# DHDev0/Stochastic-muzero

Measured on NVIDIA B200. Metric: mcts_simulations_per_sec, higher is better.
Workload: dtype bf16

## Files before the change

stochastic-muzero_b200/csrc/smz_net_bf16.cu:

```cuda
#include <cuda_bf16.h>
#include <cuda_runtime.h>
#include <stdio.h>
#include <stdlib.h>
#include <string.h>

#include "../../include/smz.h"
#include "smz_net_bf16.h"
#include "smz_tc_ptx.cuh"
#include "smz_tree_dev.cuh"

namespace {

using namespace smz_tc;

constexpr int TM = 128;
constexpr int NTHREADS = 512;
constexpr int TN = 128;
constexpr int KMAX = 128;
constexpr int MAXL = 24;
constexpr int A_BYTES = TM * KMAX * 2;
constexpr int W_BYTES = TN * KMAX * 2;
constexpr int CHUNK_A = TM * 16;
constexpr int CHUNK_W = TN * 16;
constexpr int POL_OFF = 64;
// ... 620 lines not shown
  tc_fence_before();
  __syncthreads();
  if (warp == 0) {
    asm volatile("tcgen05.dealloc.cta_group::1.sync.aligned.b32 %0, %1;" ::"r"(tmem), "r"(2 * TN) : "memory");
  }
}

template <int NT>
struct SmemPipeN {
  alignas(1024) unsigned char a[NT][A_BYTES];
  alignas(1024) unsigned char w[2][W_BYTES];
  float bias[MAXL][TN];
  unsigned long long wbar[2];
  unsigned long long dbar[NT];
  unsigned long long bbar;
  unsigned int tmem_base;
  float4 part[2][4][TM];
  int rowidx[NT][TM];
};

template <int NT>
__global__ void __launch_bounds__(NPIPE, 1)
k_bf16_chain_pipeN(SmzArena a, Chain chain0, Chain chain1, Job job, int sim) {
  extern __shared__ unsigned char smem_raw[];
  SmemPipeN<NT>& sm = *reinterpret_cast<SmemPipeN<NT>*>((reinterpret_cast<uintptr_t>(smem_raw) + 1023) & ~uintptr_t(1023));
  constexpr int NR = 2;
  const int tid = threadIdx.x, warp = tid >> 5, lane = tid & 31;
  const bool is_issuer_warp = warp == NEPI / 32;
  const int r = (warp & 3) * 32 + lane;
  const int cb = (warp >> 2) & 3;
  const int group = blockIdx.x;
  const int nl = chain0.n_layers;

  auto load_weights = [&](const Chain& c, int l, int slot) {
    const unsigned bytes = (unsigned)c.layer[l].K * TN * 2;
    mbar_expect_tx(&sm.wbar[slot], bytes);
    bulk_g2s(sm.w[slot], c.layer[l].w, bytes, &sm.wbar[slot]);
  };
  if (tid == 0) {
    mbar_init(&sm.wbar[0], 1); mbar_init(&sm.wbar[1], 1);
#pragma unroll
    for (int t = 0; t < NT; ++t) mbar_init(&sm.dbar[t], 1);
    mbar_init(&sm.bbar, 1);
    asm volatile("fence.mbarrier_init.release.cluster;" ::: "memory");
    load_weights(chain0, 0, 0);
    load_weights(chain1, 0, 1);
  }
  __syncwarp();
  if (warp == 0) {
    asm volatile("tcgen05.alloc.cta_group::1.sync.aligned.shared::cta.b32 [%0], %1;" ::"r"(s32(&sm.tmem_base)), "r"(NT * TN)
                 : "memory");
    asm volatile("tcgen05.relinquish_alloc_permit.cta_group::1.sync.aligned;" ::: "memory");
  }
  smz_pdl_wait();
  smz_pdl_launch_dependents();
  int4 rec[NT];
  uint4 hrow[NT][2];
#pragma unroll
  for (int t = 0; t < NT; ++t) { rec[t] = make_int4(0, 0, 0, 0); hrow[t][0] = hrow[t][1] = make_uint4(0, 0, 0, 0); }
  if (!is_issuer_warp) {
#pragma unroll
    for (int t = 0; t < NT; ++t) {
      const size_t ri = (size_t)(sim & 1) * a.row_cap + (size_t)(NT * group + t) * TM + r;
      rec[t] = a.rows4[ri];
      if (a.xin) {
#pragma unroll
        for (int q = 0; q < 2; ++q) hrow[t][q] = a.xin[ri * 8 + cb * 2 + q];
      } else {
        rec[t].x = min(max(rec[t].x, 0), a.B - 1);
        rec[t].y = min(max(rec[t].y, 0), a.N);
        const __nv_bfloat16* src16 = reinterpret_cast<const __nv_bfloat16*>(a.hidden) + ((size_t)rec[t].y * a.B + rec[t].x) * SMZ_SP;
#pragma unroll
        for (int q = 0; q < 2; ++q) hrow[t][q] = *reinterpret_cast<const uint4*>(src16 + (cb * 2 + q) * 8);
      }
    }
  }
  const int count0 = a.branch_count[sim * 2], count1 = a.branch_count[sim * 2 + 1];
  const int top1 = a.row_top - count1;
  const int lo = NT * group * TM;
  const int branch = lo < count0 ? 0 : (lo + NT * TM > top1 ? 1 : -1);
  if (branch < 0) {
    if (tid == 0) {
      mbar_wait(&sm.wbar[0], 0);
      mbar_wait(&sm.wbar[1], 0);
    }
    tc_fence_before();
    __syncthreads();
    tc_fence_after();
    if (warp == 0)
      asm volatile("tcgen05.dealloc.cta_group::1.sync.aligned.b32 %0, %1;" ::"r"(sm.tmem_base), "r"(NT * TN) : "memory");
    return;
  }
  unsigned actm = 0;
#pragma unroll
  for (int t = 0; t < NT; ++t)
    if (branch ? lo + (t + 1) * TM > top1 : lo + t * TM < count0) actm |= 1u << t;
  const int t_last = 31 - __clz(actm);
  const Chain& ch = branch ? chain1 : chain0;
  if (tid == 0) {
    const unsigned bbytes = (unsigned)nl * TN * 4;
    mbar_expect_tx(&sm.bbar, bbytes);
    bulk_g2s(sm.bias, ch.bias, bbytes, &sm.bbar);
  }
  tc_fence_before();
  __syncthreads();
  tc_fence_after();
  const unsigned tmem = sm.tmem_base;

  if (is_issuer_warp) {
    unsigned nfill0 = 1u, nfill1 = 1u, nseen0 = 0u, nseen1 = 0u;
    const __nv_bfloat16 *res0 = branch ? nullptr : ch.layer[0].w, *res1 = branch ? ch.layer[0].w : nullptr;
    if (nl > 1) {
      const int s1 = branch ^ 1;
      mbar_wait(&sm.wbar[s1], 0);
      if (lane == 0) load_weights(ch, 1, s1);
      if (s1) { nseen1 = 1u; nfill1 = 2u; res1 = ch.layer[1].w; } else { nseen0 = 1u; nfill0 = 2u; res0 = ch.layer[1].w; }
      __syncwarp();
    }
    for (int l = 0; l < nl; ++l) {
      const int nk = ch.layer[l].K / 16;
      const int slot = (l + branch) & 1;
      const unsigned seen = slot ? nseen1 : nseen0;
      if (seen < (slot ? nfill1 : nfill0)) {
        mbar_wait(&sm.wbar[slot], seen & 1u);
        if (slot) ++nseen1; else ++nseen0;
      }
      const unsigned long long bd = umma_desc(s32(sm.w[slot]), CHUNK_W, 128);
#pragma unroll 1
      for (int t = 0; t < NT; ++t) {
        if (!((actm >> t) & 1u)) continue;
        const unsigned long long ad = umma_desc(s32(sm.a[t]), CHUNK_A, 128);
        const unsigned d = tmem + (unsigned)(t * TN);
        for (int c = 0; c < NR; ++c) {
          nb_sync(2 + 2 * t + c);
          tc_fence_after();
          if (elect_one()) {
#pragma unroll
            for (int k = 0; k < 8; ++k)
              if (k >= 4 * c && k < 4 * (c + 1) && k < nk)
                umma(d, ad + (unsigned long long)(k * ((2 * CHUNK_A) >> 4)), bd + (unsigned long long)(k * ((2 * CHUNK_W) >> 4)),
                     k > 0 ? 1u : 0u);
          }
          __syncwarp();
        }
        if (lane == 0) umma_commit(&sm.dbar[t]);
        __syncwarp();
      }
      if (l + 2 < nl && ((slot ? res1 : res0) != ch.layer[l + 2].w || job.stream_all)) {
        mbar_wait(&sm.dbar[t_last], l & 1);
        if (lane == 0) load_weights(ch, l + 2, slot);
        if (slot) { ++nfill1; res1 = ch.layer[l + 2].w; } else { ++nfill0; res0 = ch.layer[l + 2].w; }
        __syncwarp();
      }
    }
  } else {
#pragma unroll
    for (int t = 0; t < NT; ++t) {
      const int pos = lo + t * TM + r;
      const bool tact = (actm >> t) & 1u;
      const bool valid = tact && (branch ? pos >= top1 : pos < count0);
      if (cb == 0) sm.rowidx[t][r] = valid ? rec[t].x : -1;
      if (tact) {
        const int act = valid ? rec[t].z : -1;
#pragma unroll
        for (int q = 0; q < 2; ++q) a_store(sm.a[t], r, cb * 2 + q, valid ? hrow[t][q] : make_uint4(0, 0, 0, 0));
        for (int kc = cb; kc < ch.onehot_pad / 8; kc += 4) {
          unsigned w4[4] = {0, 0, 0, 0};
          if (valid && act >= kc * 8 && act < kc * 8 + 8) {
            const int j = act - kc * 8;
            w4[j >> 1] = (j & 1) ? 0x3F800000u : 0x00003F80u;
          }
          a_store(sm.a[t], r, 8 + kc, make_uint4(w4[0], w4[1], w4[2], w4[3]));
        }
      }
    }
    fence_async_smem();
#pragma unroll
    for (int t = 0; t < NT; ++t)
      if ((actm >> t) & 1u)
        for (int c = 0; c < NR; ++c) nb_arrive(2 + 2 * t + c);
    mbar_wait(&sm.bbar, 0);
    epi_sync();
    const float (*cbias)[TN] = sm.bias;
    const int S = job.S;

    for (int l = 0; l < nl; ++l) {
      const int kind = ch.layer[l].kind;
#pragma unroll 1
      for (int t = 0; t < NT; ++t) {
        if (!((actm >> t) & 1u)) continue;
        const int index_t = sm.rowidx[t][r];
        unsigned char* const A = sm.a[t];
        const unsigned lane_t = tmem + ((unsigned)((warp & 3) * 32) << 16) + (unsigned)(t * TN);
        mbar_wait(&sm.dbar[t], l & 1);
        __syncwarp();
        tc_fence_after();
        if (kind == LK_HIDDEN) {
          constexpr int SL = 32 / NR;
          constexpr int RC = TN / NR;
          const int j0 = cb * SL;
          unsigned raw[NR][SL];
#pragma unroll
          for (int c = 0; c < NR; ++c) tmem_ld16_nowait(lane_t + c * RC + j0, raw[c]);
          tmem_wait_ld();
#pragma unroll
          for (int c = 0; c < NR; ++c) {
            const float* bias = cbias[l] + c * RC + j0;
            float x[SL];
#pragma unroll
            for (int i = 0; i < SL; ++i) x[i] = elu_fast(__uint_as_float(raw[c][i]) + bias[i]);
#pragma unroll
            for (int q = 0; q < SL / 8; ++q)
              a_store(A, r, (c * RC + j0) / 8 + q,
                      make_uint4(pack_bf16(x[q * 8 + 0], x[q * 8 + 1]), pack_bf16(x[q * 8 + 2], x[q * 8 + 3]),
                                 pack_bf16(x[q * 8 + 4], x[q * 8 + 5]), pack_bf16(x[q * 8 + 6], x[q * 8 + 7])));
            fence_async_smem();
            if (c == NR - 1) tc_fence_before();
            nb_arrive(2 + 2 * t + c);
          }
        } else {
          const int c0 = cb * 32;
          const float* bias = cbias[l] + c0;
          float4 (*part)[TM] = sm.part[t & 1];
          uint4 pend[4];
          uint4* pend_dst = nullptr;
          float x[32];
          tmem_ld32(lane_t + c0, x);
#pragma unroll
          for (int i = 0; i < 32; ++i) x[i] += bias[i];
          const bool state_seg = (kind == LK_STATE || kind == LK_STATE_REWARD) && cb < 2;
          const bool soft_seg = (kind == LK_STATE_REWARD && cb >= 2) || (kind == LK_PRED && cb < 2);
          SoftPart sp{-1e30f, 0.f, 0.f};
          if (state_seg) {
            float lo_ = INFINITY, hi_ = -INFINITY;
#pragma unroll
            for (int i = 0; i < 32; ++i) { lo_ = fminf(lo_, x[i]); hi_ = fmaxf(hi_, x[i]); }
            part[cb][r] = make_float4(lo_, hi_, 0.f, 0.f);
          } else if (soft_seg) {
            sp = soft_part(x, c0 & 63, S);
            part[cb][r] = make_float4(sp.m, sp.z, sp.y, 0.f);
          }
          epi_sync();
          if (state_seg) {
            const float4 o = part[cb ^ 1][r];
            const float lo_ = fminf(part[cb][r].x, o.x), hi_ = fmaxf(part[cb][r].y, o.y);
            float scale = hi_ - lo_;
            if (scale < 1e-5f) scale += 1e-5f;
            const float inv = 1.f / scale;
#pragma unroll
            for (int i = 0; i < 32; ++i) x[i] = (x[i] - lo_) * inv;
            if (index_t >= 0 && job.hidden16_dst) pend_dst = reinterpret_cast<uint4*>(job.hidden16_dst + (size_t)index_t * SMZ_SP + c0);
#pragma unroll
            for (int q = 0; q < 4; ++q) {
              pend[q] = make_uint4(pack_bf16(x[q * 8 + 0], x[q * 8 + 1]), pack_bf16(x[q * 8 + 2], x[q * 8 + 3]),
                                   pack_bf16(x[q * 8 + 4], x[q * 8 + 5]), pack_bf16(x[q * 8 + 6], x[q * 8 + 7]));
              a_store(A, r, cb * 4 + q, pend[q]);
            }
          } else if (soft_seg && (cb & 1) == 0) {
            const float4 o = part[cb + 1][r];
            const float v = support_scalar(sp, SoftPart{o.x, o.y, o.z});
            float* dst = (kind == LK_PRED) ? job.value_dst : job.reward_dst;
            if (index_t >= 0 && dst) dst[index_t] = v;
          } else if (kind == LK_PRED && cb == 2) {
            const int n = ch.n_policy;
            float m = -1e30f, z = 0.f;
#pragma unroll
            for (int i = 0; i < 32; ++i) m = fmaxf(m, x[i]);
#pragma unroll
            for (int i = 0; i < 32; ++i) {
              x[i] = ex2f((x[i] - m) * 1.4426950408889634f);
              z += x[i];
            }
            if (index_t >= 0 && job.policy_dst) {
              float* dst = job.policy_dst + (size_t)index_t * job.pstride;
              const float inv = 1.f / z;
#pragma unroll
              for (int i = 0; i < 32; ++i)
                if (i < n) dst[i] = x[i] * inv;
            }
          }
          if (l + 1 < nl) {
            fence_async_smem();
            tc_fence_before();
            for (int c = 0; c < NR; ++c) nb_arrive(2 + 2 * t + c);
          }
          if (pend_dst) {
#pragma unroll
            for (int q = 0; q < 4; ++q) pend_dst[q] = pend[q];
          }
        }
      }
    }
  }
  tc_fence_before();
  __syncthreads();
  if (warp == 0) {
    asm volatile("tcgen05.dealloc.cta_group::1.sync.aligned.b32 %0, %1;" ::"r"(tmem), "r"(NT * TN) : "memory");
  }
}

constexpr int TM64 = 64;
constexpr int A64_BYTES = TM64 * KMAX * 2;
constexpr int CHUNK_A64 = TM64 * 16;
constexpr unsigned IDESC64 = (1u << 4) | (1u << 7) | (1u << 10) | ((unsigned)(TN >> 3) << 17) | ((unsigned)(TM64 >> 4) << 24);

struct Smem64 {
  alignas(1024) unsigned char a[A64_BYTES];
  alignas(1024) unsigned char w[2][W_BYTES];
  float bias[2][MAXL][TN];
  unsigned long long wbar[2];
  unsigned long long dbar[2];
  unsigned long long bbar;
  unsigned int tmem_base;
  int rowidx[TM64];
  float4 part[4][TM64];
};

__device__ __forceinline__ void umma64(unsigned tmem_d, unsigned long long adesc, unsigned long long bdesc, unsigned accum) {
  asm volatile(
      "{\n\t.reg .pred p;\n\t"
      "setp.ne.b32 p, %4, 0;\n\t"
      "tcgen05.mma.cta_group::1.kind::f16 [%0], %1, %2, %3, p;\n\t}" ::"r"(tmem_d),
      "l"(adesc), "l"(bdesc), "r"(IDESC64), "r"(accum)
      : "memory");
}
__device__ __forceinline__ void a64_store2(unsigned char* a, int row, int col, unsigned v) {
  asm volatile("st.shared.b32 [%0], %1;" ::"r"(s32(a + (col >> 3) * CHUNK_A64 + row * 16 + (col & 7) * 2)), "r"(v) : "memory");
}

template <int R0, bool HALF>
__device__ __forceinline__ void chain_m64_body(const SmzArena& a, const Chain& chain0, const Chain& chain1, const Job& job, int sim) {
  extern __shared__ unsigned char smem_raw[];
  Smem64& sm = *reinterpret_cast<Smem64*>((reinterpret_cast<uintptr_t>(smem_raw) + 1023) & ~uintptr_t(1023));
  constexpr int TV = HALF ? 32 : 64;
  const int tid = threadIdx.x, warp = tid >> 5, lane = tid & 31;
  const bool is_issuer_warp = warp == NEPI / 32;
  const int q = warp & 3;
  const int cb = (warp >> 2) & 3;
  const int rA = 16 * q + (lane >> 2), rB = rA + 8;
  const int cq = 2 * (lane & 3);

  const int tile = blockIdx.x;
  const int nl = chain0.n_layers;
  long long* tl = (job.timeline && blockIdx.x == 0 && lane == 0) ? job.timeline : nullptr;
  if (tl && tid == 0) tl[0] = clock64();

  auto load_weights = [&](const Chain& c, int l, int slot) {
    const unsigned bytes = (unsigned)c.layer[l].K * TN * 2;
    mbar_expect_tx(&sm.wbar[slot], bytes);
    bulk_g2s(sm.w[slot], c.layer[l].w, bytes, &sm.wbar[slot]);
  };
  if (tid == 0) {
    mbar_init(&sm.wbar[0], 1); mbar_init(&sm.wbar[1], 1);
    mbar_init(&sm.dbar[0], 1); mbar_init(&sm.dbar[1], 1);
    mbar_init(&sm.bbar, 1);
    asm volatile("fence.mbarrier_init.release.cluster;" ::: "memory");
    const unsigned bbytes = (unsigned)nl * TN * 4;
    mbar_expect_tx(&sm.bbar, 2 * bbytes);
    bulk_g2s(sm.bias[0], chain0.bias, bbytes, &sm.bbar);
    bulk_g2s(sm.bias[1], chain1.bias, bbytes, &sm.bbar);
    load_weights(chain0, 0, 0);
    load_weights(chain1, 0, 1);
  }
  __syncwarp();
  if (warp == 0) {
    asm volatile("tcgen05.alloc.cta_group::1.sync.aligned.shared::cta.b32 [%0], %1;" ::"r"(s32(&sm.tmem_base)), "r"(2 * TN)
                 : "memory");
    asm volatile("tcgen05.relinquish_alloc_permit.cta_group::1.sync.aligned;" ::: "memory");
  }
  smz_pdl_wait();
  smz_pdl_launch_dependents();
  smz_stamp_min(a.dbg, sim, 2);
  if (tl && tid == 0) tl[1 + 4 * MAXL] = clock64();
  const bool stager = HALF ? tid < 256 : !is_issuer_warp;
  const int srow = HALF ? (tid & 31) : (tid & 63), skc = HALF ? ((tid >> 5) & 7) : ((tid >> 6) & 7);
  const int mrow = HALF ? 16 * (srow >> 3) + (srow & 7) : srow;
  const int pos = tile * TV + srow;
  int4 rec = make_int4(0, 0, 0, 0);
  uint4 hrow = make_uint4(0, 0, 0, 0);
  if (stager) {
    const size_t ri = (size_t)(sim & 1) * a.row_cap + pos;
    rec = a.rows4[ri];
    if (a.xin) {
      hrow = a.xin[ri * 8 + skc];
    } else {
      rec.x = min(max(rec.x, 0), a.B - 1);
      rec.y = min(max(rec.y, 0), a.N);
      hrow = *reinterpret_cast<const uint4*>(reinterpret_cast<const __nv_bfloat16*>(a.hidden) +
                                             ((size_t)rec.y * a.B + rec.x) * SMZ_SP + skc * 8);
    }
  }
  const int count0 = a.branch_count[sim * 2], count1 = a.branch_count[sim * 2 + 1];
  const int top1 = a.row_top - count1;
  const int branch = tile * TV < count0 ? 0 : ((tile + 1) * TV > top1 ? 1 : -1);
  if (branch < 0) {
    if (tid == 0) {
      mbar_wait(&sm.bbar, 0);
      mbar_wait(&sm.wbar[0], 0);
      mbar_wait(&sm.wbar[1], 0);
    }
    tc_fence_before();
    __syncthreads();
    tc_fence_after();
    if (warp == 0)
      asm volatile("tcgen05.dealloc.cta_group::1.sync.aligned.b32 %0, %1;" ::"r"(sm.tmem_base), "r"(2 * TN) : "memory");
    return;
  }
  const Chain& ch = branch ? chain1 : chain0;
  tc_fence_before();
  __syncthreads();
  tc_fence_after();
  const unsigned tmem = sm.tmem_base;

  if (is_issuer_warp) {
    const unsigned long long ad = umma_desc(s32(sm.a), CHUNK_A64, 128);
    unsigned nfill0 = 1u, nfill1 = 1u, nseen0 = 0u, nseen1 = 0u;
    const __nv_bfloat16 *res0 = branch ? nullptr : ch.layer[0].w, *res1 = branch ? ch.layer[0].w : nullptr;
    if (nl > 1) {
      const int s1 = branch ^ 1;
      mbar_wait(&sm.wbar[s1], 0);
      if (lane == 0) load_weights(ch, 1, s1);
      if (s1) { nseen1 = 1u; nfill1 = 2u; res1 = ch.layer[1].w; } else { nseen0 = 1u; nfill0 = 2u; res0 = ch.layer[1].w; }
      __syncwarp();
    }
    for (int l = 0; l < nl; ++l) {
      const int nk = ch.layer[l].K / 16;
      const int slot = (l + branch) & 1;
      const unsigned seen = slot ? nseen1 : nseen0;
      if (seen < (slot ? nfill1 : nfill0)) {
        mbar_wait(&sm.wbar[slot], seen & 1u);
        if (slot) ++nseen1; else ++nseen0;
      }
      const unsigned long long bd = umma_desc(s32(sm.w[slot]), CHUNK_W, 128);
      const unsigned d = tmem + (unsigned)((l & 1) * TN);
      for (int c = 0; c < 2; ++c) {
        nb_sync(2 + c);
        if (tl && c == 1) tl[1 + l * 4 + 0] = clock64();
        if (tl && c == 0 && l == 3) tl[1 + 4 * MAXL + 10] = clock64();
        tc_fence_after();
        if (elect_one()) {
#pragma unroll
          for (int k = 0; k < 8; ++k)
            if (k >= (c ? R0 / 16 : 0) && k < (c ? 8 : R0 / 16) && k < nk)
              umma64(d, ad + (unsigned long long)(k * ((2 * CHUNK_A64) >> 4)), bd + (unsigned long long)(k * ((2 * CHUNK_W) >> 4)),
                     k > 0 ? 1u : 0u);
        }
        __syncwarp();
        if (tl && c == 0 && l == 3) tl[1 + 4 * MAXL + 11] = clock64();
      }
      if (lane == 0) umma_commit(&sm.dbar[l & 1]);
      if (tl) tl[1 + l * 4 + 1] = clock64();
      __syncwarp();
      if (l + 2 < nl && ((slot ? res1 : res0) != ch.layer[l + 2].w || job.stream_all)) {
        mbar_wait(&sm.dbar[l & 1], (l >> 1) & 1);
        if (lane == 0) load_weights(ch, l + 2, slot);
        if (slot) { ++nfill1; res1 = ch.layer[l + 2].w; } else { ++nfill0; res0 = ch.layer[l + 2].w; }
        __syncwarp();
      }
    }
  } else {
    {
      if (stager) {
        const bool valid = branch ? pos >= top1 : pos < count0;
        asm volatile("st.shared.v4.b32 [%0], {%1, %2, %3, %4};" ::"r"(s32(sm.a + skc * CHUNK_A64 + mrow * 16)), "r"(valid ? hrow.x : 0u),
                     "r"(valid ? hrow.y : 0u), "r"(valid ? hrow.z : 0u), "r"(valid ? hrow.w : 0u)
                     : "memory");
        if (skc < ch.onehot_pad / 8) {
          const int act = valid ? rec.z : -1;
          unsigned w4[4] = {0, 0, 0, 0};
          if (act >= skc * 8 && act < skc * 8 + 8) {
            const int j = act - skc * 8;
            w4[j >> 1] = (j & 1) ? 0x3F800000u : 0x00003F80u;
          }
          asm volatile("st.shared.v4.b32 [%0], {%1, %2, %3, %4};" ::"r"(s32(sm.a + (8 + skc) * CHUNK_A64 + mrow * 16)), "r"(w4[0]),
                       "r"(w4[1]), "r"(w4[2]), "r"(w4[3])
                       : "memory");
        }
        if (skc == 0) sm.rowidx[mrow] = valid ? rec.x : -1;
      } else {
        const int j = tid - 256;
        const int zrow = 16 * ((j >> 3) & 3) + 8 + (j & 7), zc = j >> 5;
#pragma unroll
        for (int h = 0; h < 2; ++h)
          asm volatile("st.shared.v4.b32 [%0], {%1, %1, %1, %1};" ::"r"(s32(sm.a + (zc + 8 * h) * CHUNK_A64 + zrow * 16)), "r"(0u)
                       : "memory");
        if (zc == 0) sm.rowidx[zrow] = -1;
      }
    }
    fence_async_smem();
    for (int c = 0; c < 2; ++c) nb_arrive(2 + c);
    mbar_wait(&sm.bbar, 0);
    epi_sync();
    const unsigned lane_t = tmem + ((unsigned)(q * 32) << 16);
    const int S = job.S;
    const int idxA = sm.rowidx[rA], idxB = HALF ? -1 : sm.rowidx[rB];
    const float (*bias)[TN] = sm.bias[branch];

    for (int l = 0; l < nl; ++l) {
      const int kind = ch.layer[l].kind;
      const unsigned dcol = (unsigned)((l & 1) * TN);
      constexpr int G0 = R0 / 32, G1 = (TN - R0) / 32;
      float2 bi[G0 + G1];
      if (kind == LK_HIDDEN) {
#pragma unroll
        for (int g = 0; g < G0 + G1; ++g)
          bi[g] = *reinterpret_cast<const float2*>(bias[l] + (g < G0 ? cb * 8 * G0 + g * 8 : R0 + cb * 8 * G1 + (g - G0) * 8) + cq);
      }
      mbar_wait(&sm.dbar[l & 1], (l >> 1) & 1);
      if (tl && warp == 0) tl[1 + l * 4 + 2] = clock64();
      __syncwarp();
      tc_fence_after();
      if (kind == LK_HIDDEN) {
        unsigned raw[4 * (G0 + G1)];
        if constexpr (R0 == 64) {
          tmem_ld16x256_x2(lane_t + dcol + cb * 16, raw);
          tmem_ld16x256_x2(lane_t + dcol + 64 + cb * 16, raw + 8);
        } else {
          tmem_ld16x256_x2(lane_t + dcol + cb * 24, raw);
          tmem_ld16x256_x1(lane_t + dcol + cb * 24 + 16, raw + 8);
          tmem_ld16x256_x1(lane_t + dcol + 96 + cb * 8, raw + 12);
        }
        tmem_wait_ld();
        const bool fine = tl && warp == 0 && l == 2;
        if (fine) tl[1 + 4 * MAXL + 2] = clock64();
        unsigned pa[G0 + G1], pb[G0 + G1];
        auto math = [&](int g) {
          const unsigned* rr = raw + 4 * g;
          pa[g] = pack_bf16(elu_fast(__uint_as_float(rr[0]) + bi[g].x), elu_fast(__uint_as_float(rr[1]) + bi[g].y));
          if constexpr (!HALF) pb[g] = pack_bf16(elu_fast(__uint_as_float(rr[2]) + bi[g].x), elu_fast(__uint_as_float(rr[3]) + bi[g].y));
        };
        if constexpr (HALF) {
#pragma unroll
          for (int g = 0; g < G0 + G1; ++g) math(g);
        }
#pragma unroll
        for (int c = 0; c < 2; ++c) {
          if constexpr (!HALF) {
#pragma unroll
            for (int g = 0; g < (c ? G1 : G0); ++g) math((c ? G0 : 0) + g);
          }
#pragma unroll
          for (int g = 0; g < (c ? G1 : G0); ++g) {
            const int col = (c ? R0 + cb * 8 * G1 : cb * 8 * G0) + g * 8 + cq;
            a64_store2(sm.a, rA, col, pa[(c ? G0 : 0) + g]);
            if constexpr (!HALF) a64_store2(sm.a, rB, col, pb[(c ? G0 : 0) + g]);
          }
          if (fine) tl[1 + 4 * MAXL + 3 + 3 * c] = clock64();
          fence_async_smem();
          if (c == 1) tc_fence_before();
          if (fine) tl[1 + 4 * MAXL + 4 + 3 * c] = clock64();
          nb_arrive(2 + c);
          if (fine) tl[1 + 4 * MAXL + 5 + 3 * c] = clock64();
        }
      } else {
        const int c0 = cb * 32;
        unsigned raw[16];
        tmem_ld16x256_x4(lane_t + dcol + c0, raw);
        tmem_wait_ld();
        float xa[8], xb[8];
#pragma unroll
        for (int g = 0; g < 4; ++g) {
          const float2 bi = *reinterpret_cast<const float2*>(bias[l] + c0 + g * 8 + cq);
          xa[2 * g] = __uint_as_float(raw[4 * g + 0]) + bi.x; xa[2 * g + 1] = __uint_as_float(raw[4 * g + 1]) + bi.y;
          if constexpr (!HALF) {
            xb[2 * g] = __uint_as_float(raw[4 * g + 2]) + bi.x; xb[2 * g + 1] = __uint_as_float(raw[4 * g + 3]) + bi.y;
          } else {
            xb[2 * g] = 0.f; xb[2 * g + 1] = 0.f;
          }
        }
        const bool state_seg = (kind == LK_STATE || kind == LK_STATE_REWARD) && cb < 2;
        const bool soft_seg = (kind == LK_STATE_REWARD && cb >= 2) || (kind == LK_PRED && cb < 2);
        SoftPart spa{-1e30f, 0.f, 0.f}, spb{-1e30f, 0.f, 0.f};
        if (state_seg) {
          float loa = INFINITY, hia = -INFINITY, lob = INFINITY, hib = -INFINITY;
#pragma unroll
          for (int i = 0; i < 8; ++i) {
            loa = fminf(loa, xa[i]); hia = fmaxf(hia, xa[i]);
            if constexpr (!HALF) { lob = fminf(lob, xb[i]); hib = fmaxf(hib, xb[i]); }
          }
#pragma unroll
          for (int off = 1; off <= 2; off <<= 1) {
            loa = fminf(loa, __shfl_xor_sync(0xffffffffu, loa, off)); hia = fmaxf(hia, __shfl_xor_sync(0xffffffffu, hia, off));
            if constexpr (!HALF) {
              lob = fminf(lob, __shfl_xor_sync(0xffffffffu, lob, off)); hib = fmaxf(hib, __shfl_xor_sync(0xffffffffu, hib, off));
            }
          }
          if ((lane & 3) == 0) {
            sm.part[cb][rA] = make_float4(loa, hia, 0.f, 0.f);
            if constexpr (!HALF) sm.part[cb][rB] = make_float4(lob, hib, 0.f, 0.f);
          }
        } else if (soft_seg) {
          float ma = -1e30f, mb = -1e30f;
#pragma unroll
          for (int i = 0; i < 8; ++i) { ma = fmaxf(ma, xa[i]); if constexpr (!HALF) mb = fmaxf(mb, xb[i]); }
          spa.m = ma; spb.m = mb;
#pragma unroll
          for (int g = 0; g < 4; ++g)
#pragma unroll
            for (int j = 0; j < 2; ++j) {
              const float pos_c = (float)(((c0 + g * 8 + cq + j) & 63) - S / 2);
              const float ea = ex2f((xa[2 * g + j] - ma) * 1.4426950408889634f);
              spa.z += ea; spa.y = fmaf(pos_c, ea, spa.y);
              if constexpr (!HALF) {
                const float eb = ex2f((xb[2 * g + j] - mb) * 1.4426950408889634f);
                spb.z += eb; spb.y = fmaf(pos_c, eb, spb.y);
              }
            }
          spa = soft_quad(spa);
          if constexpr (!HALF) spb = soft_quad(spb);
          if ((lane & 3) == 0) {
            sm.part[cb][rA] = make_float4(spa.m, spa.z, spa.y, 0.f);
            if constexpr (!HALF) sm.part[cb][rB] = make_float4(spb.m, spb.z, spb.y, 0.f);
          }
        }
        epi_sync();
        unsigned pend_a[4], pend_b[4];
        bool have_pend = false;
        if (state_seg) {
          const float4 oa = sm.part[cb ^ 1][rA], ma4 = sm.part[cb][rA];
          const float loa = fminf(ma4.x, oa.x), hia = fmaxf(ma4.y, oa.y);
          float sa = hia - loa;
          if (sa < 1e-5f) sa += 1e-5f;
          const float ia = 1.f / sa;
          float lob = 0.f, ib = 0.f;
          if constexpr (!HALF) {
            const float4 ob = sm.part[cb ^ 1][rB], mb4 = sm.part[cb][rB];
            lob = fminf(mb4.x, ob.x);
            float sb = fmaxf(mb4.y, ob.y) - lob;
            if (sb < 1e-5f) sb += 1e-5f;
            ib = 1.f / sb;
          }
#pragma unroll
          for (int g = 0; g < 4; ++g) {
            pend_a[g] = pack_bf16((xa[2 * g] - loa) * ia, (xa[2 * g + 1] - loa) * ia);
            a64_store2(sm.a, rA, c0 + g * 8 + cq, pend_a[g]);
            if constexpr (!HALF) {
              pend_b[g] = pack_bf16((xb[2 * g] - lob) * ib, (xb[2 * g + 1] - lob) * ib);
              a64_store2(sm.a, rB, c0 + g * 8 + cq, pend_b[g]);
            } else {
              pend_b[g] = 0u;
            }
          }
          have_pend = job.hidden16_dst != nullptr;
        } else if (soft_seg && (cb & 1) == 0) {
          if ((lane & 3) == 0) {
            float* dst = (kind == LK_PRED) ? job.value_dst : job.reward_dst;
            if (dst) {
              const float4 oa = sm.part[cb + 1][rA];
              if (idxA >= 0) dst[idxA] = support_scalar(spa, SoftPart{oa.x, oa.y, oa.z});
              if constexpr (!HALF) {
                const float4 ob = sm.part[cb + 1][rB];
                if (idxB >= 0) dst[idxB] = support_scalar(spb, SoftPart{ob.x, ob.y, ob.z});
              }
            }
          }
        } else if (kind == LK_PRED && cb == 2) {
          const int n = ch.n_policy;
          float ma = -1e30f, mb = -1e30f;
#pragma unroll
          for (int i = 0; i < 8; ++i) { ma = fmaxf(ma, xa[i]); if constexpr (!HALF) mb = fmaxf(mb, xb[i]); }
#pragma unroll
          for (int off = 1; off <= 2; off <<= 1) {
            ma = fmaxf(ma, __shfl_xor_sync(0xffffffffu, ma, off));
            if constexpr (!HALF) mb = fmaxf(mb, __shfl_xor_sync(0xffffffffu, mb, off));
          }
          float za = 0.f, zb = 0.f;
#pragma unroll
          for (int i = 0; i < 8; ++i) {
            xa[i] = ex2f((xa[i] - ma) * 1.4426950408889634f); za += xa[i];
            if constexpr (!HALF) { xb[i] = ex2f((xb[i] - mb) * 1.4426950408889634f); zb += xb[i]; }
          }
#pragma unroll
          for (int off = 1; off <= 2; off <<= 1) {
            za += __shfl_xor_sync(0xffffffffu, za, off);
            if constexpr (!HALF) zb += __shfl_xor_sync(0xffffffffu, zb, off);
          }
          if (job.policy_dst) {
            const float ia = 1.f / za, ib = HALF ? 0.f : 1.f / zb;
#pragma unroll
            for (int g = 0; g < 4; ++g)
#pragma unroll
              for (int j = 0; j < 2; ++j) {
                const int i = g * 8 + cq + j;
                if (i < n) {
                  if (idxA >= 0) job.policy_dst[(size_t)idxA * job.pstride + i] = xa[2 * g + j] * ia;
                  if constexpr (!HALF) {
                    if (idxB >= 0) job.policy_dst[(size_t)idxB * job.pstride + i] = xb[2 * g + j] * ib;
                  }
                }
              }
          }
        }
        if (l + 1 < nl) {
          fence_async_smem();
          tc_fence_before();
          for (int c = 0; c < 2; ++c) nb_arrive(2 + c);
        }
        if (have_pend) {
#pragma unroll
          for (int g = 0; g < 4; ++g) {
            if (idxA >= 0) *reinterpret_cast<unsigned*>(job.hidden16_dst + (size_t)idxA * SMZ_SP + c0 + g * 8 + cq) = pend_a[g];
            if constexpr (!HALF) {
              if (idxB >= 0) *reinterpret_cast<unsigned*>(job.hidden16_dst + (size_t)idxB * SMZ_SP + c0 + g * 8 + cq) = pend_b[g];
            }
          }
        }
      }
      if (tl && warp == 0) tl[1 + l * 4 + 3] = clock64();
    }
  }
  tc_fence_before();
  __syncthreads();
  smz_stamp_max(a.dbg, sim, 3);
  if (warp == 0) {
    asm volatile("tcgen05.dealloc.cta_group::1.sync.aligned.b32 %0, %1;" ::"r"(tmem), "r"(2 * TN) : "memory");
  }
}

template <int R0>
__global__ void __maxnreg__(80)
k_bf16_chain_m64(SmzArena a, Chain chain0, Chain chain1, Job job, int sim) {
  chain_m64_body<R0, false>(a, chain0, chain1, job, sim);
}
__global__ void __maxnreg__(80)
k_bf16_chain_m32(SmzArena a, Chain chain0, Chain chain1, Job job, int sim) {
  chain_m64_body<96, true>(a, chain0, chain1, job, sim);
}

struct SmemMega {
  alignas(1024) unsigned char a[A_BYTES];
  alignas(1024) unsigned char w[2][2][W_BYTES];
  float bias[2][MAXL][TN];
  unsigned long long wbar[2];
  unsigned long long mbar;
  unsigned long long bbar;
  unsigned int tmem_base;
  float4 part[4][TM];
  int rowtree[TM], rowslot[TM], rowact[TM];
  int lslot[TM], lact[TM], lbranch[TM];
  int wcount[2][4];
  int n_after;
};

__global__ void __launch_bounds__(NTHREADS, 1)
k_search_mega(SmzArena a, Chain chA, Chain chD, int n_trees, int first, int n_sims, int S, long long* timeline) {
  using namespace smz_tree_dev;
  extern __shared__ unsigned char smem_raw[];
  SmemMega& sm = *reinterpret_cast<SmemMega*>((reinterpret_cast<uintptr_t>(smem_raw) + 1023) & ~uintptr_t(1023));
  const int tid = threadIdx.x, warp = tid >> 5, lane = tid & 31;
  const int r = (warp & 3) * 32 + lane;
  const int cb = warp >> 2;
  const int c0 = cb * 32;
  const int tile_base = blockIdx.x * TM;
  const int nl = chA.n_layers, total = n_sims * nl;

  auto load_weights = [&](int gl) {
    const int l = gl % nl, slot = gl & 1;
    const unsigned bytes = (unsigned)chA.layer[l].K * TN * 2;
    mbar_expect_tx(&sm.wbar[slot], 2 * bytes);
    bulk_g2s(sm.w[slot][0], chA.layer[l].w, bytes, &sm.wbar[slot]);
    bulk_g2s(sm.w[slot][1], chD.layer[l].w, bytes, &sm.wbar[slot]);
  };
  if (tid == 0) {
    mbar_init(&sm.wbar[0], 1);
    mbar_init(&sm.wbar[1], 1);
    mbar_init(&sm.mbar, 1);
    mbar_init(&sm.bbar, 1);
    asm volatile("fence.mbarrier_init.release.cluster;" ::: "memory");
    const unsigned bbytes = (unsigned)nl * TN * 4;
    mbar_expect_tx(&sm.bbar, 2 * bbytes);
    bulk_g2s(sm.bias[0], chA.bias, bbytes, &sm.bbar);
    bulk_g2s(sm.bias[1], chD.bias, bbytes, &sm.bbar);
    load_weights(0);
    if (total > 1) load_weights(1);
  }
  __syncwarp();
  if (warp == 0) {
    asm volatile("tcgen05.alloc.cta_group::1.sync.aligned.shared::cta.b32 [%0], %1;" ::"r"(s32(&sm.tmem_base)), "r"(2 * TN)
                 : "memory");
    asm volatile("tcgen05.relinquish_alloc_permit.cta_group::1.sync.aligned;" ::: "memory");
  }

  Group<4> g;
  const int ltree = tid >> 2;
  int tree = tile_base + ltree;
  const bool alive = tree < n_trees;
  if (!alive) tree = n_trees - 1;
  const SmzRng rng = smz_make_rng(a);
  TreeState ts;
  ts.cursor = a.ucursor[tree];
  ts.mm = a.minmax[tree];
  { const int4 rs = a.stat[(size_t)tree * a.M]; ts.root = make_int2(rs.x, rs.y); }

  tc_fence_before();
  __syncthreads();
  tc_fence_after();
  const unsigned tmem = sm.tmem_base;
  mbar_wait(&sm.bbar, 0);
  if (tid == 0) mbar_wait(&sm.wbar[0], 0);

  for (int it = 0; it < n_sims; ++it) {
    const int sim = first + it;
    const bool stamp = timeline && blockIdx.x == 0 && tid == 0 && it == n_sims - 1;
    if (stamp) timeline[0] = clock64();
    if (it > 0) {
      ts = expand_backup_phase(g, a, rng, tree, alive, sim - 1, a.out_policy, a.W, a.out_value, a.out_reward);
      __syncwarp();
    }
    select_phase<4, false>(g, a, rng, tree, alive, sim, ts, sm.lslot - tile_base, sm.lact - tile_base, sm.lbranch - tile_base);
    if (tid < TM) sm.rowtree[tid] = -1;
    if (stamp) timeline[1 + 4 * MAXL + 0] = clock64();
    __syncthreads();
    if (stamp) timeline[1 + 4 * MAXL + 1] = clock64();
    unsigned m0 = 0, m1 = 0;
    int mybranch = 2;
    if (tid < TM) {
      if (tile_base + tid < n_trees) mybranch = sm.lbranch[tid];
      m0 = __ballot_sync(0xffffffffu, mybranch == 0);
      m1 = __ballot_sync(0xffffffffu, mybranch == 1);
      if (lane == 0) { sm.wcount[0][warp] = __popc(m0); sm.wcount[1][warp] = __popc(m1); }
    }
    __syncthreads();
    if (tid < TM) {
      int n0 = 0, pre0 = 0, pre1 = 0;
      for (int w2 = 0; w2 < 4; ++w2) {
        if (w2 < warp) { pre0 += sm.wcount[0][w2]; pre1 += sm.wcount[1][w2]; }
        n0 += sm.wcount[0][w2];
      }
      const unsigned lt = (1u << lane) - 1u;
      if (mybranch < 2) {
        const int pos = mybranch == 0 ? pre0 + __popc(m0 & lt) : n0 + pre1 + __popc(m1 & lt);
        sm.rowtree[pos] = tile_base + tid;
        sm.rowslot[pos] = sm.lslot[tid];
        sm.rowact[pos] = sm.lact[tid];
      }
      if (tid == 0) sm.n_after = n0;
    }
    __syncthreads();
    const int index = sm.rowtree[r];
    const int n_after = sm.n_after;
    const int br = r >= n_after;
    {
      const bool valid = index >= 0;
      const __nv_bfloat16* src16 = valid
          ? reinterpret_cast<const __nv_bfloat16*>(a.hidden) + ((size_t)sm.rowslot[r] * a.B + index) * SMZ_SP : nullptr;
      const int act = valid ? sm.rowact[r] : -1;
#pragma unroll
      for (int q = 0; q < 2; ++q) {
        const int kc = cb * 2 + q;
        a_store(sm.a, r, kc, valid ? *reinterpret_cast<const uint4*>(src16 + kc * 8) : make_uint4(0, 0, 0, 0));
      }
      for (int kc = cb; kc < chA.onehot_pad / 8; kc += 4) {
        unsigned w4[4] = {0, 0, 0, 0};
        if (valid && act >= kc * 8 && act < kc * 8 + 8) {
          const int j = act - kc * 8;
          w4[j >> 1] = (j & 1) ? 0x3F800000u : 0x00003F80u;
        }
        a_store(sm.a, r, 8 + kc, make_uint4(w4[0], w4[1], w4[2], w4[3]));
      }
    }
    fence_async_smem();
    tc_fence_before();
    __syncthreads();
    if (stamp) timeline[1 + 4 * MAXL + 2] = clock64();
    const int q0 = (warp & 3) * 32;
    const bool mixed = n_after > q0 && n_after < q0 + 32;
    const unsigned taddr0 = tmem + ((unsigned)q0 << 16) + (unsigned)c0;

    for (int l = 0; l < nl; ++l) {
      const int gl = it * nl + l;
      const int K = chA.layer[l].K;
      const int kindA = chA.layer[l].kind;
      if (tid == 0) {
        if (stamp) timeline[1 + l * 4 + 0] = clock64();
        tc_fence_after();
        const unsigned long long ad = umma_desc(s32(sm.a), CHUNK_A, 128);
        const int nk = K / 16;
#pragma unroll
        for (int net = 0; net < 2; ++net) {
          const unsigned long long bd = umma_desc(s32(sm.w[gl & 1][net]), CHUNK_W, 128);
          umma(tmem + net * TN, ad, bd, 0u);
#pragma unroll
          for (int k = 1; k < 8; ++k)
            if (k < nk)
              umma(tmem + net * TN, ad + (unsigned long long)(k * ((2 * CHUNK_A) >> 4)),
                   bd + (unsigned long long)(k * ((2 * CHUNK_W) >> 4)), 1u);
        }
        umma_commit(&sm.mbar);
        if (stamp) timeline[1 + l * 4 + 1] = clock64();
        if (gl + 1 < total) mbar_wait(&sm.wbar[(gl + 1) & 1], ((gl + 1) >> 1) & 1);
      }
      mbar_wait(&sm.mbar, gl & 1);
      __syncwarp();
      if (stamp) timeline[1 + l * 4 + 2] = clock64();
      tc_fence_after();
      if (tid == 0 && gl + 2 < total) load_weights(gl + 2);
      __syncwarp();
      const float* bias = sm.bias[br][l] + c0;

      uint4 pend[4];
      uint4* pend_dst = nullptr;
      float x[32];
      if (!mixed) {
        tmem_ld32(taddr0 + (unsigned)(br * TN), x);
      } else {
        float y[32];
        tmem_ld32(taddr0, x);
        tmem_ld32(taddr0 + TN, y);
#pragma unroll
        for (int j = 0; j < 32; ++j) x[j] = br ? y[j] : x[j];
      }
#pragma unroll
      for (int j = 0; j < 32; ++j) x[j] += bias[j];

      if (kindA == LK_HIDDEN) {
#pragma unroll
        for (int j = 0; j < 32; ++j) x[j] = elu_fast(x[j]);
#pragma unroll
        for (int q = 0; q < 4; ++q)
          a_store(sm.a, r, cb * 4 + q,
                  make_uint4(pack_bf16(x[q * 8 + 0], x[q * 8 + 1]), pack_bf16(x[q * 8 + 2], x[q * 8 + 3]),
                             pack_bf16(x[q * 8 + 4], x[q * 8 + 5]), pack_bf16(x[q * 8 + 6], x[q * 8 + 7])));
      } else {
        const bool is_pred = kindA == LK_PRED;
        const bool state_seg = !is_pred && cb < 2;
        const bool soft_seg = (is_pred && cb < 2) || (!is_pred && br == 1 && cb >= 2);
        SoftPart sp{-1e30f, 0.f, 0.f};
        if (state_seg) {
          float lo = INFINITY, hi = -INFINITY;
#pragma unroll
          for (int j = 0; j < 32; ++j) { lo = fminf(lo, x[j]); hi = fmaxf(hi, x[j]); }
          sm.part[cb][r] = make_float4(lo, hi, 0.f, 0.f);
        } else if (soft_seg) {
          sp = soft_part(x, c0 & 63, S);
          sm.part[cb][r] = make_float4(sp.m, sp.z, sp.y, 0.f);
        }
        __syncthreads();
        if (state_seg) {
          const float4 o = sm.part[cb ^ 1][r];
          const float lo = fminf(sm.part[cb][r].x, o.x), hi = fmaxf(sm.part[cb][r].y, o.y);
          float scale = hi - lo;
          if (scale < 1e-5f) scale += 1e-5f;
          const float inv = 1.f / scale;
#pragma unroll
          for (int j = 0; j < 32; ++j) x[j] = (x[j] - lo) * inv;
          if (index >= 0)
            pend_dst = reinterpret_cast<uint4*>(reinterpret_cast<__nv_bfloat16*>(a.hidden) +
                                                ((size_t)(sim + 1) * a.B + index) * SMZ_SP + c0);
#pragma unroll
          for (int q = 0; q < 4; ++q) {
            pend[q] = make_uint4(pack_bf16(x[q * 8 + 0], x[q * 8 + 1]), pack_bf16(x[q * 8 + 2], x[q * 8 + 3]),
                                 pack_bf16(x[q * 8 + 4], x[q * 8 + 5]), pack_bf16(x[q * 8 + 6], x[q * 8 + 7]));
            a_store(sm.a, r, cb * 4 + q, pend[q]);
          }
        } else if (soft_seg && (cb & 1) == 0) {
          const float4 o = sm.part[cb + 1][r];
          const float v = support_scalar(sp, SoftPart{o.x, o.y, o.z});
          if (index >= 0) (is_pred ? a.out_value : a.out_reward)[index] = v;
        } else if (is_pred && cb == 2) {
          const int n = br ? chD.n_policy : chA.n_policy;
          float m = -1e30f, z = 0.f;
#pragma unroll
          for (int i = 0; i < 32; ++i) m = fmaxf(m, x[i]);
#pragma unroll
          for (int i = 0; i < 32; ++i) {
            x[i] = ex2f((x[i] - m) * 1.4426950408889634f);
            z += x[i];
          }
          if (index >= 0) {
            float* dst = a.out_policy + (size_t)index * a.W;
            const float inv = 1.f / z;
#pragma unroll
            for (int i = 0; i < 32; ++i)
              if (i < n) dst[i] = x[i] * inv;
          }
        }
      }
      fence_async_smem();
      tc_fence_before();
      __syncthreads();
      if (pend_dst) {
#pragma unroll
        for (int q = 0; q < 4; ++q) pend_dst[q] = pend[q];
      }
      if (stamp) timeline[1 + l * 4 + 3] = clock64();
    }
  }
  expand_backup_phase(g, a, rng, tree, alive, first + n_sims - 1, a.out_policy, a.W, a.out_value, a.out_reward);
  tc_fence_before();
  __syncthreads();
  if (warp == 0) {
    asm volatile("tcgen05.dealloc.cta_group::1.sync.aligned.b32 %0, %1;" ::"r"(tmem), "r"(2 * TN) : "memory");
  }
}

__global__ void k_pack_bf16(__nv_bfloat16* __restrict__ dst, const float* __restrict__ src, int n_rows, int in_stride,
                            int seg0, int seg1_dst, int seg1_src, int seg1_n, int dst_n0) {
// ... 318 lines not shown
```

stochastic-muzero_b200/csrc/smz_tc_ptx.cuh:

```cuda
#pragma once
#include <cuda_bf16.h>
#include <cuda_runtime.h>
#include <stdio.h>

namespace smz_tc {

__device__ __forceinline__ unsigned s32(const void* p) { return (unsigned)__cvta_generic_to_shared(p); }

__device__ __forceinline__ void mbar_init(unsigned long long* bar, unsigned count) {
  asm volatile("mbarrier.init.shared::cta.b64 [%0], %1;" ::"r"(s32(bar)), "r"(count));
}
__device__ __forceinline__ void mbar_expect_tx(unsigned long long* bar, unsigned bytes) {
  asm volatile("mbarrier.arrive.expect_tx.shared::cta.b64 _, [%0], %1;" ::"r"(s32(bar)), "r"(bytes) : "memory");
}
__device__ __forceinline__ void mbar_wait(unsigned long long* bar, unsigned parity) {
  const unsigned addr = s32(bar);
#pragma unroll 1
  for (unsigned spin = 0; spin < (1u << 26); ++spin) {
    unsigned ok;
    asm volatile(
        "{\n\t.reg .pred p;\n\t"
        "mbarrier.try_wait.parity.shared::cta.b64 p, [%1], %2;\n\t"
        "selp.u32 %0, 1, 0, p;\n\t}"
        : "=r"(ok)
        : "r"(addr), "r"(parity)
        : "memory");
    if (ok) return;
  }
  printf("smz bf16: mbarrier wait timed out (block %d thread %d)\n", blockIdx.x, threadIdx.x);
  __trap();
}
__device__ __forceinline__ void bulk_g2s(void* dst, const void* src, unsigned bytes, unsigned long long* bar) {
  asm volatile("cp.async.bulk.shared::cluster.global.mbarrier::complete_tx::bytes [%0], [%1], %2, [%3];" ::"r"(s32(dst)),
               "l"(src), "r"(bytes), "r"(s32(bar))
               : "memory");
}
__device__ __forceinline__ void fence_async_smem() { asm volatile("fence.proxy.async.shared::cta;" ::: "memory"); }
__device__ __forceinline__ void tc_fence_before() { asm volatile("tcgen05.fence::before_thread_sync;" ::: "memory"); }
__device__ __forceinline__ void tc_fence_after() { asm volatile("tcgen05.fence::after_thread_sync;" ::: "memory"); }

__device__ __forceinline__ unsigned long long umma_desc(unsigned smem_addr, unsigned lbo_bytes, unsigned sbo_bytes) {
  return (unsigned long long)((smem_addr & 0x3FFFFu) >> 4) | ((unsigned long long)(lbo_bytes >> 4) << 16) |
         ((unsigned long long)(sbo_bytes >> 4) << 32) | (1ull << 46);
}

__device__ __forceinline__ bool elect_one() {
  unsigned pred;
  asm volatile(
      "{\n\t.reg .pred p;\n\t"
      "elect.sync _|p, 0xffffffff;\n\t"
      "selp.u32 %0, 1, 0, p;\n\t}"
      : "=r"(pred));
  return pred != 0;
}
__device__ __forceinline__ void umma_commit(unsigned long long* bar) {
  asm volatile("tcgen05.commit.cta_group::1.mbarrier::arrive::one.shared::cluster.b64 [%0];" ::"r"(s32(bar)) : "memory");
}
__device__ __forceinline__ void tmem_ld32(unsigned taddr, float* v) {
  unsigned r[32];
  asm volatile(
      "tcgen05.ld.sync.aligned.32x32b.x32.b32 "
      "{%0, %1, %2, %3, %4, %5, %6, %7, %8, %9, %10, %11, %12, %13, %14, %15, "
      "%16, %17, %18, %19, %20, %21, %22, %23, %24, %25, %26, %27, %28, %29, %30, %31}, [%32];"
      : "=r"(r[0]), "=r"(r[1]), "=r"(r[2]), "=r"(r[3]), "=r"(r[4]), "=r"(r[5]), "=r"(r[6]), "=r"(r[7]), "=r"(r[8]),
        "=r"(r[9]), "=r"(r[10]), "=r"(r[11]), "=r"(r[12]), "=r"(r[13]), "=r"(r[14]), "=r"(r[15]), "=r"(r[16]),
        "=r"(r[17]), "=r"(r[18]), "=r"(r[19]), "=r"(r[20]), "=r"(r[21]), "=r"(r[22]), "=r"(r[23]), "=r"(r[24]),
        "=r"(r[25]), "=r"(r[26]), "=r"(r[27]), "=r"(r[28]), "=r"(r[29]), "=r"(r[30]), "=r"(r[31])
      : "r"(taddr)
      : "memory");
  asm volatile("tcgen05.wait::ld.sync.aligned;" ::: "memory");
#pragma unroll
  for (int i = 0; i < 32; ++i) v[i] = __uint_as_float(r[i]);
}

__device__ __forceinline__ void tmem_ld16_nowait(unsigned taddr, unsigned* r) {
  asm volatile(
      "tcgen05.ld.sync.aligned.32x32b.x16.b32 "
      "{%0, %1, %2, %3, %4, %5, %6, %7, %8, %9, %10, %11, %12, %13, %14, %15}, [%16];"
      : "=r"(r[0]), "=r"(r[1]), "=r"(r[2]), "=r"(r[3]), "=r"(r[4]), "=r"(r[5]), "=r"(r[6]), "=r"(r[7]), "=r"(r[8]),
        "=r"(r[9]), "=r"(r[10]), "=r"(r[11]), "=r"(r[12]), "=r"(r[13]), "=r"(r[14]), "=r"(r[15])
      : "r"(taddr)
      : "memory");
}
__device__ __forceinline__ void tmem_wait_ld() { asm volatile("tcgen05.wait::ld.sync.aligned;" ::: "memory"); }

__device__ __forceinline__ unsigned pack_bf16(float lo, float hi) {
  __nv_bfloat162 p = __floats2bfloat162_rn(lo, hi);
  return *reinterpret_cast<unsigned*>(&p);
}

__device__ __forceinline__ float ex2f(float x) {
  float y;
  asm("ex2.approx.ftz.f32 %0, %1;" : "=f"(y) : "f"(x));
  return y;
}

struct SoftPart { float m, z, y; };
__device__ __forceinline__ SoftPart soft_part(const float* x, int col0, int S) {
  SoftPart p{-1e30f, 0.f, 0.f};
#pragma unroll
  for (int i = 0; i < 32; ++i) p.m = fmaxf(p.m, x[i]);
  const float base = (float)(col0 - S / 2);
#pragma unroll
  for (int i = 0; i < 32; ++i) {
    const float e = ex2f((x[i] - p.m) * 1.4426950408889634f);
    p.z += e;
    p.y = fmaf(base + (float)i, e, p.y);
  }
  return p;
}
__device__ __forceinline__ float support_scalar(SoftPart a, SoftPart b) {
  const float m = fmaxf(a.m, b.m);
  const float sa = ex2f((a.m - m) * 1.4426950408889634f);
  const float sb = ex2f((b.m - m) * 1.4426950408889634f);
  const float y = (a.y * sa + b.y * sb) / (a.z * sa + b.z * sb);
  const float inner = __fadd_rn(1.f, __fmul_rn(0.004f, __fadd_rn(__fadd_rn(fabsf(y), 1.f), 0.001f)));
  const float t = __fdiv_rn(__fsub_rn(__fsqrt_rn(inner), 1.f), 0.002f);
  const float mag = __fsub_rn(__fmul_rn(t, t), 1.f);
  return y > 0.f ? mag : (y < 0.f ? -mag : 0.f);
}

__device__ __forceinline__ void tmem_ld8_nowait(unsigned taddr, unsigned* r) {
  asm volatile("tcgen05.ld.sync.aligned.32x32b.x8.b32 {%0, %1, %2, %3, %4, %5, %6, %7}, [%8];"
               : "=r"(r[0]), "=r"(r[1]), "=r"(r[2]), "=r"(r[3]), "=r"(r[4]), "=r"(r[5]), "=r"(r[6]), "=r"(r[7])
               : "r"(taddr)
               : "memory");
}

__device__ __forceinline__ void tmem_ld16x256_x2(unsigned taddr, unsigned* r) {
  asm volatile("tcgen05.ld.sync.aligned.16x256b.x2.b32 {%0, %1, %2, %3, %4, %5, %6, %7}, [%8];"
               : "=r"(r[0]), "=r"(r[1]), "=r"(r[2]), "=r"(r[3]), "=r"(r[4]), "=r"(r[5]), "=r"(r[6]), "=r"(r[7])
               : "r"(taddr)
               : "memory");
}
__device__ __forceinline__ void tmem_ld16x256_x1(unsigned taddr, unsigned* r) {
  asm volatile("tcgen05.ld.sync.aligned.16x256b.x1.b32 {%0, %1, %2, %3}, [%4];"
               : "=r"(r[0]), "=r"(r[1]), "=r"(r[2]), "=r"(r[3])
               : "r"(taddr)
               : "memory");
}
__device__ __forceinline__ void tmem_ld16x256_x4(unsigned taddr, unsigned* r) {
  asm volatile(
      "tcgen05.ld.sync.aligned.16x256b.x4.b32 {%0, %1, %2, %3, %4, %5, %6, %7, %8, %9, %10, %11, %12, %13, %14, %15}, [%16];"
      : "=r"(r[0]), "=r"(r[1]), "=r"(r[2]), "=r"(r[3]), "=r"(r[4]), "=r"(r[5]), "=r"(r[6]), "=r"(r[7]), "=r"(r[8]),
        "=r"(r[9]), "=r"(r[10]), "=r"(r[11]), "=r"(r[12]), "=r"(r[13]), "=r"(r[14]), "=r"(r[15])
      : "r"(taddr)
      : "memory");
}

__device__ __forceinline__ SoftPart soft_merge(SoftPart a, SoftPart b) {
  const float m = fmaxf(a.m, b.m);
  const float sa = ex2f((a.m - m) * 1.4426950408889634f), sb = ex2f((b.m - m) * 1.4426950408889634f);
  return SoftPart{m, a.z * sa + b.z * sb, a.y * sa + b.y * sb};
}
__device__ __forceinline__ SoftPart soft_quad(SoftPart p) {
#pragma unroll
  for (int off = 1; off <= 2; off <<= 1) {
    SoftPart o{__shfl_xor_sync(0xffffffffu, p.m, off), __shfl_xor_sync(0xffffffffu, p.z, off), __shfl_xor_sync(0xffffffffu, p.y, off)};
    p = soft_merge(p, o);
  }
  return p;
}

}
```

Baseline: 180.6 million.

## Keep inter-layer activations in tensor memory and use TMEM-sourced A operand MMAs

In the M64 chain path, activations produced by the epilogue for layers after the first are written to tensor memory with tcgen05.st instead of shared memory. The MMA issuer then uses the tcgen05.mma form that takes A from TMEM. The accumulator now always sits in one TMEM column range, with the A operand in the next range, replacing the previous ping-pong of accumulator columns. This removes shared-memory stores and async-proxy fences between layers. In exchange, accumulator double-buffering is lost, so the epilogue's TMEM reads and the next layer's MMA must serialize, and the TMEM A-operand layout has to match what the MMA expects.

```diff
diff --git a/stochastic-muzero_b200/csrc/smz_net_bf16.cu b/stochastic-muzero_b200/csrc/smz_net_bf16.cu
--- a/stochastic-muzero_b200/csrc/smz_net_bf16.cu
+++ b/stochastic-muzero_b200/csrc/smz_net_bf16.cu
@@ -946,6 +946,7 @@
 constexpr int TM64 = 64;
 constexpr int A64_BYTES = TM64 * KMAX * 2;
 constexpr int CHUNK_A64 = TM64 * 16;
+constexpr unsigned A64_TCOL = TN;
 constexpr unsigned IDESC64 = (1u << 4) | (1u << 7) | (1u << 10) | ((unsigned)(TN >> 3) << 17) | ((unsigned)(TM64 >> 4) << 24);
 
 struct Smem64 {
@@ -968,8 +969,22 @@
       "l"(adesc), "l"(bdesc), "r"(IDESC64), "r"(accum)
       : "memory");
 }
-__device__ __forceinline__ void a64_store2(unsigned char* a, int row, int col, unsigned v) {
-  asm volatile("st.shared.b32 [%0], %1;" ::"r"(s32(a + (col >> 3) * CHUNK_A64 + row * 16 + (col & 7) * 2)), "r"(v) : "memory");
+template <int N>
+__device__ __forceinline__ void a64_tstore(unsigned taddr, const unsigned* pa, const unsigned* pb) {
+  unsigned r[2 * N];
+#pragma unroll
+  for (int i = 0; i < N; ++i) { r[2 * i] = pa[i]; r[2 * i + 1] = pb[i]; }
+  if constexpr (N == 1) {
+    tmem_st16x128_x1(taddr, r[0], r[1]);
+  } else if constexpr (N == 2) {
+    tmem_st16x128_x2(taddr, r);
+  } else if constexpr (N == 3) {
+    tmem_st16x128_x2(taddr, r);
+    tmem_st16x128_x1(taddr + 8, r[4], r[5]);
+  } else {
+    static_assert(N == 4, "a64_tstore: 1 .. 4 groups");
+    tmem_st16x128_x4(taddr, r);
+  }
 }
 
 template <int R0, bool HALF>
@@ -1076,7 +1091,6 @@
         if (slot) ++nseen1; else ++nseen0;
       }
       const unsigned long long bd = umma_desc(s32(sm.w[slot]), CHUNK_W, 128);
-      const unsigned d = tmem + (unsigned)((l & 1) * TN);
       for (int c = 0; c < 2; ++c) {
         nb_sync(2 + c);
         if (tl && c == 1) tl[1 + l * 4 + 0] = clock64();
@@ -1085,9 +1099,13 @@
         if (elect_one()) {
 #pragma unroll
           for (int k = 0; k < 8; ++k)
-            if (k >= (c ? R0 / 16 : 0) && k < (c ? 8 : R0 / 16) && k < nk)
-              umma64(d, ad + (unsigned long long)(k * ((2 * CHUNK_A64) >> 4)), bd + (unsigned long long)(k * ((2 * CHUNK_W) >> 4)),
-                     k > 0 ? 1u : 0u);
+            if (k >= (c ? R0 / 16 : 0) && k < (c ? 8 : R0 / 16) && k < nk) {
+              const unsigned long long bk = bd + (unsigned long long)(k * ((2 * CHUNK_W) >> 4));
+              if (l == 0)
+                umma64(tmem, ad + (unsigned long long)(k * ((2 * CHUNK_A64) >> 4)), bk, k > 0 ? 1u : 0u);
+              else
+                umma_ts(tmem, tmem + A64_TCOL + 8 * k, bk, IDESC64, k > 0 ? 1u : 0u);
+            }
         }
         __syncwarp();
         if (tl && c == 0 && l == 3) tl[1 + 4 * MAXL + 11] = clock64();
@@ -1135,14 +1153,13 @@
     for (int c = 0; c < 2; ++c) nb_arrive(2 + c);
     mbar_wait(&sm.bbar, 0);
     epi_sync();
-    const unsigned lane_t = tmem + ((unsigned)(q * 32) << 16);
+    const unsigned lane_t = tmem + ((unsigned)(q * 32) << 16), a_t = lane_t + A64_TCOL;
     const int S = job.S;
     const int idxA = sm.rowidx[rA], idxB = HALF ? -1 : sm.rowidx[rB];
     const float (*bias)[TN] = sm.bias[branch];
 
     for (int l = 0; l < nl; ++l) {
       const int kind = ch.layer[l].kind;
-      const unsigned dcol = (unsigned)((l & 1) * TN);
       constexpr int G0 = R0 / 32, G1 = (TN - R0) / 32;
       float2 bi[G0 + G1];
       if (kind == LK_HIDDEN) {
@@ -1157,12 +1174,12 @@
       if (kind == LK_HIDDEN) {
         unsigned raw[4 * (G0 + G1)];
         if constexpr (R0 == 64) {
-          tmem_ld16x256_x2(lane_t + dcol + cb * 16, raw);
-          tmem_ld16x256_x2(lane_t + dcol + 64 + cb * 16, raw + 8);
+          tmem_ld16x256_x2(lane_t + cb * 16, raw);
+          tmem_ld16x256_x2(lane_t + 64 + cb * 16, raw + 8);
         } else {
-          tmem_ld16x256_x2(lane_t + dcol + cb * 24, raw);
-          tmem_ld16x256_x1(lane_t + dcol + cb * 24 + 16, raw + 8);
-          tmem_ld16x256_x1(lane_t + dcol + 96 + cb * 8, raw + 12);
+          tmem_ld16x256_x2(lane_t + cb * 24, raw);
+          tmem_ld16x256_x1(lane_t + cb * 24 + 16, raw + 8);
+          tmem_ld16x256_x1(lane_t + 96 + cb * 8, raw + 12);
         }
         tmem_wait_ld();
         const bool fine = tl && warp == 0 && l == 2;
@@ -1172,6 +1189,7 @@
           const unsigned* rr = raw + 4 * g;
           pa[g] = pack_bf16(elu_fast(__uint_as_float(rr[0]) + bi[g].x), elu_fast(__uint_as_float(rr[1]) + bi[g].y));
           if constexpr (!HALF) pb[g] = pack_bf16(elu_fast(__uint_as_float(rr[2]) + bi[g].x), elu_fast(__uint_as_float(rr[3]) + bi[g].y));
+          else pb[g] = 0u;
         };
         if constexpr (HALF) {
 #pragma unroll
@@ -1183,15 +1201,13 @@
 #pragma unroll
             for (int g = 0; g < (c ? G1 : G0); ++g) math((c ? G0 : 0) + g);
           }
-#pragma unroll
-          for (int g = 0; g < (c ? G1 : G0); ++g) {
-            const int col = (c ? R0 + cb * 8 * G1 : cb * 8 * G0) + g * 8 + cq;
-            a64_store2(sm.a, rA, col, pa[(c ? G0 : 0) + g]);
-            if constexpr (!HALF) a64_store2(sm.a, rB, col, pb[(c ? G0 : 0) + g]);
-          }
+          if (c == 0)
+            a64_tstore<G0>(a_t + cb * 4 * G0, pa, pb);
+          else
+            a64_tstore<G1>(a_t + R0 / 2 + cb * 4 * G1, pa + G0, pb + G0);
           if (fine) tl[1 + 4 * MAXL + 3 + 3 * c] = clock64();
-          fence_async_smem();
-          if (c == 1) tc_fence_before();
+          tmem_wait_st();
+          tc_fence_before();
           if (fine) tl[1 + 4 * MAXL + 4 + 3 * c] = clock64();
           nb_arrive(2 + c);
           if (fine) tl[1 + 4 * MAXL + 5 + 3 * c] = clock64();
@@ -1199,7 +1215,7 @@
       } else {
         const int c0 = cb * 32;
         unsigned raw[16];
-        tmem_ld16x256_x4(lane_t + dcol + c0, raw);
+        tmem_ld16x256_x4(lane_t + c0, raw);
         tmem_wait_ld();
         float xa[8], xb[8];
 #pragma unroll
@@ -1277,14 +1293,10 @@
 #pragma unroll
           for (int g = 0; g < 4; ++g) {
             pend_a[g] = pack_bf16((xa[2 * g] - loa) * ia, (xa[2 * g + 1] - loa) * ia);
-            a64_store2(sm.a, rA, c0 + g * 8 + cq, pend_a[g]);
-            if constexpr (!HALF) {
-              pend_b[g] = pack_bf16((xb[2 * g] - lob) * ib, (xb[2 * g + 1] - lob) * ib);
-              a64_store2(sm.a, rB, c0 + g * 8 + cq, pend_b[g]);
-            } else {
-              pend_b[g] = 0u;
-            }
-          }
+            if constexpr (!HALF) pend_b[g] = pack_bf16((xb[2 * g] - lob) * ib, (xb[2 * g + 1] - lob) * ib);
+            else pend_b[g] = 0u;
+          }
+          a64_tstore<4>(a_t + c0 / 2, pend_a, pend_b);
           have_pend = job.hidden16_dst != nullptr;
         } else if (soft_seg && (cb & 1) == 0) {
           if ((lane & 3) == 0) {
@@ -1336,7 +1348,7 @@
           }
         }
         if (l + 1 < nl) {
-          fence_async_smem();
+          tmem_wait_st();
           tc_fence_before();
           for (int c = 0; c < 2; ++c) nb_arrive(2 + c);
         }
diff --git a/stochastic-muzero_b200/csrc/smz_tc_ptx.cuh b/stochastic-muzero_b200/csrc/smz_tc_ptx.cuh
--- a/stochastic-muzero_b200/csrc/smz_tc_ptx.cuh
+++ b/stochastic-muzero_b200/csrc/smz_tc_ptx.cuh
@@ -52,6 +52,14 @@
       "selp.u32 %0, 1, 0, p;\n\t}"
       : "=r"(pred));
   return pred != 0;
+}
+__device__ __forceinline__ void umma_ts(unsigned tmem_d, unsigned tmem_a, unsigned long long bdesc, unsigned idesc, unsigned accum) {
+  asm volatile(
+      "{\n\t.reg .pred p;\n\t"
+      "setp.ne.b32 p, %4, 0;\n\t"
+      "tcgen05.mma.cta_group::1.kind::f16 [%0], [%1], %2, %3, p;\n\t}" ::"r"(tmem_d),
+      "r"(tmem_a), "l"(bdesc), "r"(idesc), "r"(accum)
+      : "memory");
 }
 __device__ __forceinline__ void umma_commit(unsigned long long* bar) {
   asm volatile("tcgen05.commit.cta_group::1.mbarrier::arrive::one.shared::cluster.b64 [%0];" ::"r"(s32(bar)) : "memory");
@@ -148,6 +156,21 @@
       : "memory");
 }
 
+__device__ __forceinline__ void tmem_st16x128_x1(unsigned taddr, unsigned r0, unsigned r1) {
+  asm volatile("tcgen05.st.sync.aligned.16x128b.x1.b32 [%0], {%1, %2};" ::"r"(taddr), "r"(r0), "r"(r1) : "memory");
+}
+__device__ __forceinline__ void tmem_st16x128_x2(unsigned taddr, const unsigned* r) {
+  asm volatile("tcgen05.st.sync.aligned.16x128b.x2.b32 [%0], {%1, %2, %3, %4};" ::"r"(taddr), "r"(r[0]), "r"(r[1]), "r"(r[2]),
+               "r"(r[3])
+               : "memory");
+}
+__device__ __forceinline__ void tmem_st16x128_x4(unsigned taddr, const unsigned* r) {
+  asm volatile("tcgen05.st.sync.aligned.16x128b.x4.b32 [%0], {%1, %2, %3, %4, %5, %6, %7, %8};" ::"r"(taddr), "r"(r[0]), "r"(r[1]),
+               "r"(r[2]), "r"(r[3]), "r"(r[4]), "r"(r[5]), "r"(r[6]), "r"(r[7])
+               : "memory");
+}
+__device__ __forceinline__ void tmem_wait_st() { asm volatile("tcgen05.wait::st.sync.aligned;" ::: "memory"); }
+
 __device__ __forceinline__ SoftPart soft_merge(SoftPart a, SoftPart b) {
   const float m = fmaxf(a.m, b.m);
   const float sa = ex2f((a.m - m) * 1.4426950408889634f), sb = ex2f((b.m - m) * 1.4426950408889634f);
```

After: 186.8 million, median of 6. 3.4% higher.
